# traveller59/second.pytorch

Measured on AMD Instinct MI355X. Metric: frames/sec VoxelNet fwd (car.fhd, ~16k active voxels), higher is better.
Workload: dtype bf16; 1 GPU; car.fhd.config VoxelNet forward (voxelise+VFE+SpMiddleFHD+RPNV2+rotated NMS), inference, batch=8 synthetic KITTI clouds/GPU (17000 pts, 16000 voxels each), random-init weights, inputs resident in HBM; parallelism=frame-dp1, launch_mode=graph, graph_branches=1, steps_in_flight=4, rpn_segments_serialized=True, rulebook_numbering=sorted, points_per_frame=17000

## Files before the change

second.pytorch_amd/csrc/dense.hip:

```cpp
#include "common.hpp"
#include <type_traits>
#include <stdio.h>
#include <stdlib.h>
#include <stdlib.h>

namespace sec {

template <typename T> __device__ __forceinline__ float to_f(T v);
template <> __device__ __forceinline__ float to_f(__hip_bfloat16 v) { return __bfloat162float(v); }
template <> __device__ __forceinline__ float to_f(__half v) { return __half2float(v); }
template <typename T> __device__ __forceinline__ T from_f(float v);
template <> __device__ __forceinline__ __hip_bfloat16 from_f(float v) { return __float2bfloat16(v); }
template <> __device__ __forceinline__ __half from_f(float v) { return __float2half_rn(v); }

template <typename T>
__global__ __launch_bounds__(kBlock) void k_bias_act16(T *__restrict__ x, const float *__restrict__ bias, long long n_vec,
                                                      int c_vec, int relu) {
    for (long long g = (long long)blockIdx.x * kBlock + threadIdx.x; g < n_vec; g += (long long)gridDim.x * kBlock) {
        uint4 v = reinterpret_cast<uint4 *>(x)[g];
        T *e = reinterpret_cast<T *>(&v);
        const float *b = bias + (size_t)(g % c_vec) * 8;
#pragma unroll
        for (int i = 0; i < 8; ++i) {
            float f = to_f<T>(e[i]) + b[i];
// ... 7 lines not shown
__global__ __launch_bounds__(kBlock) void k_bias_act32(float *__restrict__ x, const float *__restrict__ bias, long long n_vec,
                                                      int c_vec, int relu) {
    for (long long g = (long long)blockIdx.x * kBlock + threadIdx.x; g < n_vec; g += (long long)gridDim.x * kBlock) {
        float4 v = reinterpret_cast<float4 *>(x)[g];
        const float *b = bias + (size_t)(g % c_vec) * 4;
        v.x += b[0]; v.y += b[1]; v.z += b[2]; v.w += b[3];
        if (relu) { v.x = fmaxf(v.x, 0.f); v.y = fmaxf(v.y, 0.f); v.z = fmaxf(v.z, 0.f); v.w = fmaxf(v.w, 0.f); }
        reinterpret_cast<float4 *>(x)[g] = v;
    }
}

typedef float f32x16d __attribute__((ext_vector_type(16)));
typedef __bf16 bf16x8d __attribute__((ext_vector_type(8)));
typedef _Float16 f16x8d __attribute__((ext_vector_type(8)));
template <typename T> struct MfmaD;
template <> struct MfmaD<__hip_bfloat16> {
    static __device__ __forceinline__ f32x16d run(uint4 a, uint4 b, f32x16d c) {
        return __builtin_amdgcn_mfma_f32_32x32x16_bf16(__builtin_bit_cast(bf16x8d, a), __builtin_bit_cast(bf16x8d, b), c, 0, 0, 0);
    }
};
template <> struct MfmaD<__half> {
    static __device__ __forceinline__ f32x16d run(uint4 a, uint4 b, f32x16d c) {
        return __builtin_amdgcn_mfma_f32_32x32x16_f16(__builtin_bit_cast(f16x8d, a), __builtin_bit_cast(f16x8d, b), c, 0, 0, 0);
    }
};


typedef float f32x2d __attribute__((ext_vector_type(2)));
template <typename T> __device__ __forceinline__ unsigned pack2(float a, float b);
template <> __device__ __forceinline__ unsigned pack2<__hip_bfloat16>(float a, float b) {
    typedef __bf16 bf16x2d __attribute__((ext_vector_type(2)));
    const f32x2d v = {a, b};
    return __builtin_bit_cast(unsigned, __builtin_convertvector(v, bf16x2d));
}
template <> __device__ __forceinline__ unsigned pack2<__half>(float a, float b) {
    typedef _Float16 f16x2d __attribute__((ext_vector_type(2)));
    const f32x2d v = {a, b};
    return __builtin_bit_cast(unsigned, __builtin_convertvector(v, f16x2d));
}

template <typename T> __device__ __forceinline__ uint2 pack4(float a, float b, float c, float d) {
    T t[4] = {from_f<T>(a), from_f<T>(b), from_f<T>(c), from_f<T>(d)};
    uint2 u;
    __builtin_memcpy(&u, t, 8);
    return u;
}
// ... 184 lines not shown
#pragma unroll
        for (int mt = 0; mt < 2; ++mt) {
            const long long pix0 = m0 + wm * 64 + mt * 32 + 4 * hh;
            T *yp = y + (size_t)pix0 * ldc + co;
#pragma unroll
            for (int i = 0; i < 16; ++i) {
                const int ro = (i & 3) + 8 * (i >> 2);
                if (pix0 + ro < p.m) {
                    float v = acc[mt][nt][i] + bv;
                    if (p.relu) v = v > 0.0f ? v : 0.0f;
                    yp[(size_t)ro * ldc] = from_f<T>(v);
                }
            }
        }
    }
}

template <int N> __device__ __forceinline__ void wait_vmcnt() { asm volatile("s_waitcnt vmcnt(%0)" ::"n"(N) : "memory"); }
__device__ __forceinline__ void lds_barrier() { asm volatile("s_waitcnt lgkmcnt(0)\n\ts_barrier" ::: "memory"); }

template <int CH, int HW_, bool COLKEY> __device__ __forceinline__ int halo_key(int hp) {
    return (COLKEY && CH == 16) ? ((hp % HW_) & 15) : (hp & (CH - 1));
}

#ifdef SEC_CONV2D_EXPERIMENTS
#include "../../tools/kernel_experiments/dense_conv2d_ab.inc"
#endif

template <typename T, int CIN, int TH, int ROLL = 0, bool GATHER = false, int NSPLIT = 1, bool X3 = false, bool TAIL = false>
__global__ __launch_bounds__(256, CIN == 128 ? 3 : 2) void k_conv2d_halo_reg(const T *__restrict__ x, const T *__restrict__ wpk,
                                                            const float *__restrict__ bias, T *__restrict__ y,
                                                            Conv2dParams p, int tiles_y, int tiles_x, int per_xcd,
                                                            const int *__restrict__ site_map, unsigned feat_bytes,
                                                            const unsigned short *__restrict__ tile_order = nullptr,
                                                            const int *__restrict__ live_counts = nullptr,
                                                            const T *__restrict__ background = nullptr,
                                                            const unsigned short *__restrict__ nbr_masks = nullptr,
                                                            const T *__restrict__ bg_in = nullptr,
                                                            const T *__restrict__ x_lo = nullptr, T *__restrict__ y_lo = nullptr,
                                                            const T *__restrict__ background_lo = nullptr,
                                                            const T *__restrict__ bg_in_lo = nullptr, ConvTailArgs tail = ConvTailArgs{}) {
    static_assert(!GATHER || (ROLL == 2 && CIN == 128), "gather prologue: the shared-row loop on two 64-channel planes");
    static_assert(!TAIL || (ROLL == 2 && CIN == 128 && TH == 8 && !GATHER && NSPLIT == 1 && !X3), "fused 1x1 tail: the lazy list form of the 128-channel conv");
    static_assert(!X3 || (ROLL == 2 && CIN == 128 && TH == 8 && !GATHER && NSPLIT == 1 && std::is_same<T, __hip_bfloat16>::value),
                  "three-pass split-fp32 form: the shared-row bf16 loop");
    constexpr int TW = 16, HW_ = TW + 2, HPIX = (TH + 2) * (TW + 2);
    static_assert(NSPLIT == 1 || (NSPLIT == 2 && ROLL == 0 && !GATHER), "pixel split: the two-stage loop only");
    constexpr int MT = TH * TW / 32 / NSPLIT;
    constexpr int CH = CIN / 8, HENT = HPIX * CH;
    constexpr int KC = CIN / 64, NIT = 9 * KC;
    extern __shared__ __attribute__((aligned(16))) uint4 halo_smem[];
    uint4 *hal = halo_smem;
    const int tid = threadIdx.x, lane = tid & 63, wv = tid >> 6;
    const int r = lane & 31, hh = lane >> 5;
    const int ntile = p.batch * tiles_y * tiles_x;
    const int xcd = blockIdx.x % 8, local = blockIdx.x / 8;
    const int n0 = blockIdx.y * (128 / NSPLIT) + (wv % (4 / NSPLIT)) * 32;
    const int mtb = (wv / (4 / NSPLIT)) * MT;
    constexpr int cin8 = CIN / 8;
    const uint4 *x4 = reinterpret_cast<const uint4 *>(x);
    const uint4 *w4 = reinterpret_cast<const uint4 *>(wpk);
    const uint4 *zero16 = w4 + (size_t)9 * cin8 * p.cout;
    auto issue_halo = [&](int tile) {
        const int b = tile / (tiles_y * tiles_x);
        const int trem = tile - b * tiles_y * tiles_x;
        const int y0 = (trem / tiles_x) * TH, x0 = (trem % tiles_x) * TW;
        for (int i = wv; i < (HENT + 63) / 64; i += 4) {
// ... 2 lines not shown
            const int hp = e / CH, slot = e - hp * CH;
            const int hy = hp / HW_, hx = hp - hy * HW_;
            const int iy = y0 - 1 + hy, ix = x0 - 1 + hx;
            const bool ok = iy >= 0 && iy < p.h && ix >= 0 && ix < p.w;
            const uint4 *src = ok ? x4 + (((long long)b * p.h + iy) * p.w + ix) * cin8 + (slot ^ halo_key<CH, HW_, true>(hp)) : zero16;
            __builtin_amdgcn_global_load_lds((glb_ptr_t)src, (lds_ptr_t)&hal[i * 64], 16, 0, 0);
        }
    };
    auto issue_halo2 = [&](int tile, const T *xsrc) {
        const int b = tile / (tiles_y * tiles_x);
        const int trem = tile - b * tiles_y * tiles_x;
        const int y0 = (trem / tiles_x) * TH, x0 = (trem % tiles_x) * TW;
        const unsigned img_bytes = (unsigned)p.h * (unsigned)p.w * (CIN * 2u);
        const __amdgpu_buffer_rsrc_t xrs = __builtin_amdgcn_make_buffer_rsrc(const_cast<T *>(xsrc) + (size_t)b * p.h * p.w * CIN, 0, (int)img_bytes, 0x00020000);
        const int wvs = __builtin_amdgcn_readfirstlane(wv);
        const unsigned slot = lane & 15;
        const unsigned row_pitch = (unsigned)p.w * (CIN * 2u);
        int hx = wvs * 4 + (lane >> 4);
        unsigned rowoff = (unsigned)((y0 - 1) * p.w + (x0 - 1)) * (CIN * 2u);
#pragma unroll
        for (int t = 0; t < (HENT / 64 + 3) / 4; ++t) {
            const int i = wvs + 4 * t;
            if (i < HENT / 64) {
                const unsigned key = (slot ^ ((unsigned)hx & 15u)) << 4;
                unsigned off = rowoff + ((unsigned)hx << 8) + key;
                const unsigned ix = (unsigned)(x0 - 1 + hx);
                off = ix < (unsigned)p.w ? off : 0xfffffff0u;
                __builtin_amdgcn_raw_ptr_buffer_load_lds(xrs, (lds_ptr_t)&hal[i * 64], 16, off, 0, 0, 0);
            }
            hx += 16;
            const bool wrap = hx >= HW_;
            hx = wrap ? hx - HW_ : hx;
            rowoff = wrap ? rowoff + row_pitch : rowoff;
        }
    };
    auto issue_halo2_lazy = [&](int tile, unsigned nmask, const T *xsrc, const T *bgsrc) {
        const int b = tile / (tiles_y * tiles_x);
        const int trem = tile - b * tiles_y * tiles_x;
        const int y0 = (trem / tiles_x) * TH, x0 = (trem % tiles_x) * TW;
        const unsigned img_bytes = (unsigned)p.h * (unsigned)p.w * (CIN * 2u);
        const __amdgpu_buffer_rsrc_t xrs = __builtin_amdgcn_make_buffer_rsrc(const_cast<T *>(xsrc) + (size_t)b * p.h * p.w * CIN, 0, (int)img_bytes, 0x00020000);
        const __amdgpu_buffer_rsrc_t ers = __builtin_amdgcn_make_buffer_rsrc(const_cast<T *>(bgsrc), 0, (int)img_bytes, 0x00020000);
        const int wvs = __builtin_amdgcn_readfirstlane(wv);
        const unsigned slot = lane & 15;
        const unsigned row_pitch = (unsigned)p.w * (CIN * 2u);
        int hx = wvs * 4 + (lane >> 4), hy = 0;
        unsigned rowoff = (unsigned)((y0 - 1) * p.w + (x0 - 1)) * (CIN * 2u);
#pragma unroll
        for (int t = 0; t < (HENT / 64 + 3) / 4; ++t) {
            const int i = wvs + 4 * t;
            if (i < HENT / 64) {
                const unsigned key = (slot ^ ((unsigned)hx & 15u)) << 4;
                unsigned off = rowoff + ((unsigned)hx << 8) + key;
                const unsigned ix = (unsigned)(x0 - 1 + hx);
                off = ix < (unsigned)p.w ? off : 0xfffffff0u;
                const int ry = hy == 0 ? 0 : (hy == TH + 1 ? 2 : 1), rx = hx == 0 ? 0 : (hx == HW_ - 1 ? 2 : 1);
                if ((nmask >> (ry * 3 + rx)) & 1u) __builtin_amdgcn_raw_ptr_buffer_load_lds(xrs, (lds_ptr_t)&hal[i * 64], 16, off, 0, 0, 0);
                else __builtin_amdgcn_raw_ptr_buffer_load_lds(ers, (lds_ptr_t)&hal[i * 64], 16, off, 0, 0, 0);
            }
            hx += 16;
            const bool wrap = hx >= HW_;
            hx = wrap ? hx - HW_ : hx;
            hy = wrap ? hy + 1 : hy;
            rowoff = wrap ? rowoff + row_pitch : rowoff;
        }
    };
    auto issue_halo_gather = [&](int tile) -> unsigned {
        constexpr int NP = (HENT / 64 + 3) / 4;
        const int b = tile / (tiles_y * tiles_x);
        const int trem = tile - b * tiles_y * tiles_x;
        const int y0 = (trem / tiles_x) * TH, x0 = (trem % tiles_x) * TW;
        const unsigned plane = (unsigned)p.h * (unsigned)p.w;
        const __amdgpu_buffer_rsrc_t mrs = __builtin_amdgcn_make_buffer_rsrc(const_cast<int *>(site_map) + (size_t)b * 2 * plane, 0, (int)(plane * 8u), 0x00020000);
        const __amdgpu_buffer_rsrc_t frs = __builtin_amdgcn_make_buffer_rsrc(const_cast<T *>(x), 0, (int)feat_bytes, 0x00020000);
        const int wvs = __builtin_amdgcn_readfirstlane(wv);
        const unsigned slot = lane & 15;
        int hx = wvs * 4 + (lane >> 4), iy = y0 - 1;
        unsigned rowp1[NP], coff[NP], any = 0;
#pragma unroll
        for (int t = 0; t < NP; ++t) {
            const int i = wvs + 4 * t;
            rowp1[t] = 0;
            coff[t] = 0;
            if (i < HENT / 64) {
                const unsigned c = slot ^ ((unsigned)hx & 15u);
                const int ix = x0 - 1 + hx;
                const bool ok = (unsigned)ix < (unsigned)p.w && (unsigned)iy < (unsigned)p.h;
                const unsigned moff = ((c >> 3 ? plane : 0u) + (unsigned)(iy * p.w + ix)) * 4u;
                rowp1[t] = __builtin_amdgcn_raw_buffer_load_b32(mrs, ok ? moff : 0xfffffffcu, 0, 0);
                coff[t] = (c & 7u) << 4;
            }
            hx += 16;
            const bool wrap = hx >= HW_;
            hx = wrap ? hx - HW_ : hx;
            iy = wrap ? iy + 1 : iy;
        }
#pragma unroll
        for (int t = 0; t < NP; ++t) any |= rowp1[t];
        __shared__ unsigned wave_any[4];
        const unsigned long long bal = __ballot(any != 0);
        if (lane == 0) wave_any[wv] = bal != 0ull;
        __syncthreads();
        if ((wave_any[0] | wave_any[1] | wave_any[2] | wave_any[3]) == 0u) return 0u;
#pragma unroll
        for (int t = 0; t < NP; ++t) {
            const int i = wvs + 4 * t;
            if (i < HENT / 64) {
                const unsigned off = rowp1[t] ? (rowp1[t] - 1u) * (CIN * 1u) + coff[t] : 0xfffffff0u;
// ... 141 lines not shown
            for (int ty_ = 0; ty_ < TH; ++ty_) {
                const int oy = y0 + ty_;
                if (oy < p.h && ox < p.w) y4[(((size_t)b * p.h + oy) * p.w + ox) * (p.cout / 8) + blockIdx.y * 16 + ch] = v;
            }
            return;
        }
    } else if constexpr (ROLL >= 2) {
        if (nbr_masks) issue_halo2_lazy(tile, nmask, x, bg_in);
        else issue_halo2(tile, x);
    } else issue_halo(tile);
#ifdef SEC_CONV_TIMELINE
    long long tl_issue = 0, tl_eb1 = 0, tl_eb2 = 0;
    if (tl) tl_issue = clock64();
#endif
    {
        const int b = tile / (tiles_y * tiles_x);
        const int trem = tile - b * tiles_y * tiles_x;
        const int y0 = (trem / tiles_x) * TH, x0 = (trem % tiles_x) * TW;
        uint4 bq[2][4];
        constexpr int RD = 8;
        uint4 br[RD];
        typedef unsigned int u32x4b __attribute__((ext_vector_type(4)));
        const __amdgpu_buffer_rsrc_t wrs = __builtin_amdgcn_make_buffer_rsrc(const_cast<T *>(wpk), 0, (int)(((X3 ? 18 : 9) * cin8 + 1) * p.cout * 16), 0x00020000);
        const unsigned wvoff = (unsigned)(hh * p.cout + n0 + r) * 16u;
        const unsigned wstep = (unsigned)p.cout * 16u;
        auto ld_b = [&](unsigned chunk) {
            return __builtin_bit_cast(uint4, (u32x4b)__builtin_amdgcn_raw_buffer_load_b128(wrs, wvoff, chunk * wstep, 0));
        };
        if constexpr (ROLL >= 2) {
#pragma unroll
            for (int f = 0; f < RD - 1; ++f) br[f] = ld_b((f % 3) * 48 + (f / 3) * 2);
        } else if constexpr (ROLL) {
#pragma unroll
            for (int f = 0; f < RD - 1; ++f) br[f] = wlane[(size_t)f * 2 * p.cout];
        } else {
            load_b(0, bq[0]);
        }
        f32x16d acc[MT];
#pragma unroll
        for (int a = 0; a < MT; ++a)
#pragma unroll
            for (int i = 0; i < 16; ++i) acc[a][i] = 0.0f;
        __syncthreads();
#ifdef SEC_CONV_TIMELINE
        if (tl) tl1 = clock64();
#endif
        bool live = true;
        if constexpr (GATHER) live = gather_live != 0;
        else if (p.zskip) {
            unsigned nz = 0;
            for (int e = tid; e < HENT; e += 256) {
                const uint4 v = hal[e];
                nz |= v.x | v.y | v.z | v.w;
            }
            live = __syncthreads_or((int)(nz != 0)) != 0;
        }
        uint4 af[2][MT];
        int tap = 0, kc = 0;
        if (live && !ROLL) load_a(0, 0, 0, af[0]);
        if constexpr (ROLL >= 2) {
            static_assert(ROLL < 2 || (KC == 2 && CH == 16 && TH == 8), "8 k-steps per tap, rows (mt, mt + 4)");
            const char *halb = reinterpret_cast<const char *>(hal);
            const int colr = r & 15;
            const unsigned base0 = (unsigned)((r >> 4) * 4 * HW_ + colr) * (CH * 16);
            uint4 fr[2][6];
            auto load_f2 = [&](unsigned bdx, unsigned key, int cidx, int j0, uint4 (&dst)[6]) {
                const unsigned a = bdx + (((unsigned)cidx << 4) ^ key);
#pragma unroll
                for (int j = j0; j < j0 + 2; ++j) dst[j] = *reinterpret_cast<const uint4 *>(halb + a + j * HW_ * (CH * 16));
            };
            auto frag_off = [](int j) { return (j % 3) * 48 + (j / 3) * 2; };
            if (live) {
                constexpr int NPASS = X3 ? 3 : 1;
#pragma unroll 1
                for (int pass = 0; pass < NPASS; ++pass) {
                    const unsigned wp = (X3 && pass == 1) ? 9u * cin8 : 0u;
                    if (X3 && pass > 0) {
                        if (pass == 2) {
                            __syncthreads();
                            if (nbr_masks) issue_halo2_lazy(tile, nmask, x_lo, bg_in_lo);
                            else issue_halo2(tile, x_lo);
                        }
#pragma unroll
// ... 73 lines not shown
            if (nkc == KC) { nkc = 0; ++ntap; }
#pragma unroll
            for (int s = 0; s < 4; ++s) {
                if (s < 3) load_a(tap, kc, s + 1, af[(s + 1) & 1]);
                else if (it + 1 < NIT) load_a(ntap, nkc, 0, af[0]);
#pragma unroll
                for (int mt = 0; mt < MT; ++mt) acc[mt] = MfmaD<T>::run(bq[cur][s], af[s & 1][mt], acc[mt]);
            }
            tap = ntap;
            kc = nkc;
        }
#ifdef SEC_CONV_TIMELINE
        if (tl) tl2 = clock64();
#endif
        if constexpr (CIN == 128 && TH == 8) {
            constexpr int PITCH = 17;
            __syncthreads();
#ifdef SEC_CONV_TIMELINE
            if (tl) tl_eb1 = clock64();
#endif
            uint4 *ot = halo_smem;
            float4 bv[4];
#pragma unroll
            for (int g = 0; g < 4; ++g) bv[g] = bias ? *reinterpret_cast<const float4 *>(bias + n0 + 8 * g + 4 * hh) : make_float4(0.0f, 0.0f, 0.0f, 0.0f);
            auto put_tile = [&](auto relu_tag, auto lo_tag) {
                constexpr bool RELU = decltype(relu_tag)::value;
                constexpr bool LOW = decltype(lo_tag)::value;
#pragma unroll
                for (int mt = 0; mt < MT; ++mt) {
                    unsigned lo[4], hi[4];
#pragma unroll
                    for (int g = 0; g < 4; ++g) {
                        float v[4] = {acc[mt][4 * g] + bv[g].x, acc[mt][4 * g + 1] + bv[g].y, acc[mt][4 * g + 2] + bv[g].z, acc[mt][4 * g + 3] + bv[g].w};
                        if (RELU) {
#pragma unroll
                            for (int j = 0; j < 4; ++j) v[j] = __builtin_fmaxf(v[j], 0.0f);
                        }
                        lo[g] = pack2<T>(v[0], v[1]);
                        hi[g] = pack2<T>(v[2], v[3]);
                        if constexpr (LOW) {
                            lo[g] = pack2<T>(v[0] - __uint_as_float(lo[g] << 16), v[1] - __uint_as_float(lo[g] & 0xffff0000u));
                            hi[g] = pack2<T>(v[2] - __uint_as_float(hi[g] << 16), v[3] - __uint_as_float(hi[g] & 0xffff0000u));
                        }
                    }
                    const int q = ROLL >= 2 ? (mt + 4 * (r >> 4)) * 16 + (r & 15) : mt * 32 + r;
#pragma unroll
                    for (int pr = 0; pr < 2; ++pr) {
                        const auto sx = __builtin_amdgcn_permlane32_swap(lo[2 * pr], lo[2 * pr + 1], false, false);
                        const auto sy = __builtin_amdgcn_permlane32_swap(hi[2 * pr], hi[2 * pr + 1], false, false);
                        ot[q * PITCH + wv * 4 + 2 * pr + hh] = make_uint4(sx[0], sy[0], sx[1], sy[1]);
// ... 150 lines not shown
                                  const unsigned short *nbr_masks = nullptr, const void *bg_in = nullptr,
                                  const void *x_lo = nullptr, void *y_lo = nullptr, const void *background_lo = nullptr,
                                  const void *bg_in_lo = nullptr, const ConvTailArgs &tail = ConvTailArgs{}) {
    constexpr size_t lds_tile = (size_t)(TH + 2) * 18 * (CIN / 8) * 16;
    const long lds_pad = 0;
    const size_t lds = lds_tile + (size_t)lds_pad;
    static bool configured = false;
    auto fn = k_conv2d_halo_reg<T, CIN, TH, ROLL, GATHER, NSPLIT, X3, TAIL>;
    if (!configured) {
        (void)hipFuncSetAttribute(reinterpret_cast<const void *>(fn), hipFuncAttributeMaxDynamicSharedMemorySize, (int)lds);
        configured = true;
    }
    const int ty = div_up(p.h, TH), tx = div_up(p.w, 16);
    const int per_xcd = div_up(p.batch * ty * tx, 8);
    const int gx = per_xcd * 8;
    if (TAIL) set_last_kernel("k_conv2d_halo_reg<%s, %d, %d, %d, false, 1, false, true>", dtype_name<T>(), CIN, TH, ROLL);
    else if (X3) set_last_kernel("k_conv2d_halo_reg<%s, %d, %d, %d, false, 1, true>", dtype_name<T>(), CIN, TH, ROLL);
    else if (NSPLIT == 1) set_last_kernel("k_conv2d_halo_reg<%s, %d, %d, %d, %s>", dtype_name<T>(), CIN, TH, ROLL, GATHER ? "true" : "false");
    else set_last_kernel("k_conv2d_halo_reg<%s, %d, %d, %d, %s, %d>", dtype_name<T>(), CIN, TH, ROLL, GATHER ? "true" : "false", NSPLIT);
    hipLaunchKernelGGL(fn, dim3(gx, p.cout / (128 / NSPLIT)), dim3(256), lds, st, (const T *)x, (const T *)wpk, bias, (T *)y, p, ty, tx, per_xcd,
                       site_map, feat_bytes, tile_order, live_counts, (const T *)background, nbr_masks, (const T *)bg_in, (const T *)x_lo, (T *)y_lo,
                       (const T *)background_lo, (const T *)bg_in_lo, tail);
    return check_launch();
}

template <typename T, int BN, int TPW>
__global__ __launch_bounds__(kBlock) void k_conv1x1_nhwc(const T *__restrict__ x, const T *__restrict__ wpk,
                                                        const float *__restrict__ bias, T *__restrict__ y, Conv2dParams p) {
    constexpr int BM = 128, NTW = BN / 64, CC = 2;
    constexpr int PERB = BN * 8 / kBlock;
    __shared__ uint4 sA[2][BM * 8];
    __shared__ uint4 sB[CC][8 * BN];
    const int tid = threadIdx.x, lane = tid & 63, wv = tid >> 6;
    const int r = lane & 31, hh = lane >> 5;
    const int wm = wv & 1, wn = wv >> 1;
    const int n0 = blockIdx.y * BN;
    const int cin8 = p.cin / 8;
    const uint4 *x4 = reinterpret_cast<const uint4 *>(x);
    const uint4 *w4 = reinterpret_cast<const uint4 *>(wpk);
    const uint4 *zero16 = w4 + (size_t)cin8 * p.cout;
    const long long tile0 = (long long)blockIdx.x * TPW;
    const long long ntiles = (p.m + BM - 1) / BM;
    if (tile0 >= ntiles) return;
    const int nt_local = (int)((ntiles - tile0 < TPW) ? ntiles - tile0 : TPW);
    const int slot = lane & 7;
    auto issue_a = [&](int it, int buf) {
// ... 390 lines not shown
}

#include "dense_patch.hpp"

static bool conv2d_patch_enabled() {
    static int v = -1;
    if (v < 0) {
        const char *e = getenv("SEC_CONV2D_PATCH");
        v = (e && *e == '0') ? 0 : 1;
    }
    return v != 0;
}

template <typename T>
static int launch_conv2d(const void *x, const void *wpk, const float *bias, void *y, const Conv2dParams &p, hipStream_t st) {
    dim3 block(kBlock);
    if (conv2d_variant() == 13 && conv2d_patch_enabled()) {
        const int rc = patch::dispatch<T>(x, wpk, bias, y, p, p.cout, st);
        if (rc != patch::kNotTaken) return rc;
    }
    if (conv2d_variant() == 14 && p.ksize == 3 && p.stride == 1 && p.pad == 1 && p.cout % 128 == 0 && p.cin == 128)
        return launch_conv2d_halo_reg<T, 128, 8>(x, wpk, bias, y, p, st);
    if (conv2d_variant() == 13 && p.ksize == 3 && p.stride == 1 && p.pad == 1 && p.cout % 128 == 0 && (p.cin == 128 || p.cin == 64))
        return p.cin == 128 ? launch_conv2d_halo_reg<T, 128, 8, 2>(x, wpk, bias, y, p, st) : launch_conv2d_halo_reg<T, 64, 8>(x, wpk, bias, y, p, st);
    if (conv2d_variant() == 13 && p.ksize == 3 && p.stride == 1 && p.pad == 1 && p.cout % 128 == 0 && p.cin == 256)
        return launch_conv2d_halo_reg<T, 256, 4>(x, wpk, bias, y, p, st);
    if (conv2d_variant() == 13 && p.ksize == 3 && p.stride == 1 && p.pad == 1 && p.cout == 64 && p.cin == 64)
        return launch_conv2d_halo_reg<T, 64, 8, 0, false, 2>(x, wpk, bias, y, p, st);
    if (conv2d_variant() == 15 && p.ksize == 3 && p.stride == 1 && p.pad == 1 && p.cout % 128 == 0 && p.cin == 128)
        return launch_conv2d_halo_reg<T, 128, 8, 1>(x, wpk, bias, y, p, st);
#ifdef SEC_CONV2D_EXPERIMENTS
    if (conv2d_variant() >= 5 && conv2d_variant() <= 12 && p.ksize == 3 && p.stride == 1 && p.pad == 1 && p.cout % 128 == 0 &&
        (p.cin == 128 || p.cin == 64)) {
#define SEC_HALO_PIPE(NQ_, KS_, NB_, CK_, FP_)                                                                  \
    return p.cin == 128 ? launch_conv2d_halo_pipe<T, 128, 8, NQ_, KS_, NB_, CK_, FP_>(x, wpk, bias, y, p, st)   \
                        : launch_conv2d_halo_pipe<T, 64, 8, NQ_, KS_, NB_, CK_, FP_>(x, wpk, bias, y, p, st)
        switch (conv2d_variant()) {
        case 5: SEC_HALO_PIPE(4, 64, 2, false, false);
        case 8: SEC_HALO_PIPE(2, 64, 2, true, false);
        case 10: SEC_HALO_PIPE(4, 64, 2, true, false);
        case 11: SEC_HALO_PIPE(4, 64, 2, false, true);
        default: SEC_HALO_PIPE(4, 64, 2, true, true);
        }
#undef SEC_HALO_PIPE
    }
    if (conv2d_variant() >= 2 && conv2d_variant() <= 4 && p.ksize == 3 && p.stride == 1 && p.pad == 1 &&
        p.cout % 128 == 0 && (p.cin == 128 || p.cin == 64)) {
// ... 200 lines not shown
                              void *workspace, size_t workspace_bytes, void *stream) {
    return rpn_tile_live_impl(site_map, batch, h, w, layers, tile_order, live_counts, nullptr, workspace, workspace_bytes, stream);
}

SEC_API int sec_rpn_tile_live_masks(const int *site_map, int batch, int h, int w, int layers, unsigned short *tile_order, int *live_counts,
                                    unsigned short *nbr_masks, void *workspace, size_t workspace_bytes, void *stream) {
    if (!nbr_masks) return SEC_E_INVALID;
    return rpn_tile_live_impl(site_map, batch, h, w, layers, tile_order, live_counts, nbr_masks, workspace, workspace_bytes, stream);
}

static int conv2d_tiles_impl(const void *x, int batch, int h, int w, const void *packed_weight, const float *bias, int cout, int relu,
                             const unsigned short *tile_order, const int *live_counts, const void *background,
                             const unsigned short *nbr_masks, const void *background_in, void *y, int dtype, void *stream) {
    if (!x || !packed_weight || !y || batch <= 0 || h <= 0 || w <= 0 || (tile_order && !live_counts)) return SEC_E_INVALID;
    if (cout % 128 || (dtype != SEC_BF16 && dtype != SEC_F16)) return SEC_E_UNSUPPORTED;
    apply_list_threshold_env();
    Conv2dParams p;
    p.batch = batch; p.h = h; p.w = w; p.cin = 128; p.cout = cout; p.ksize = 3; p.stride = 1; p.pad = 1;
    p.relu = relu & 1; p.zskip = 0; p.stagger = 0;
    p.ho = h; p.wo = w;
    p.m = (long long)batch * h * w;
    hipStream_t st = (hipStream_t)stream;
    if (dtype == SEC_BF16)
        return launch_conv2d_halo_reg<__hip_bfloat16, 128, 8, 2>(x, packed_weight, bias, y, p, st, nullptr, 0, tile_order, live_counts, background,
                                                                 nbr_masks, background_in);
    return launch_conv2d_halo_reg<__half, 128, 8, 2>(x, packed_weight, bias, y, p, st, nullptr, 0, tile_order, live_counts, background, nbr_masks,
                                                     background_in);
}

SEC_API int sec_conv2d_nhwc_tiles(const void *x, int batch, int h, int w, const void *packed_weight, const float *bias, int cout,
                                  int relu, const unsigned short *tile_order, const int *live_counts, const void *background,
                                  void *y, int dtype, void *stream) {
    if (tile_order && !background) return SEC_E_INVALID;
    return conv2d_tiles_impl(x, batch, h, w, packed_weight, bias, cout, relu, tile_order, live_counts, background, nullptr, nullptr, y, dtype,
                             stream);
}

SEC_API int sec_conv2d_nhwc_tiles_lazy(const void *x, int batch, int h, int w, const void *packed_weight, const float *bias, int cout,
                                       int relu, const unsigned short *tile_order, const int *live_counts, const void *background,
                                       const unsigned short *nbr_masks, const void *background_in, void *y, int dtype, void *stream) {
    if (!tile_order || !nbr_masks || !background_in) return SEC_E_INVALID;
    return conv2d_tiles_impl(x, batch, h, w, packed_weight, bias, cout, relu, tile_order, live_counts, background, nbr_masks, background_in, y,
                             dtype, stream);
}

SEC_API int sec_conv2d_nhwc_tiles_tail(const void *x, int batch, int h, int w, const void *packed_weight, const float *bias, int relu,
                                       const unsigned short *tile_order, const int *live_counts, const unsigned short *nbr_masks,
                                       const void *background_in, const void *packed_w1, const float *bias1, int relu1, const void *packed_w2,
                                       const float *bias2, int cout2, void *y_heads, int dtype, void *stream) {
    if (!x || !packed_weight || !tile_order || !live_counts || !nbr_masks || !background_in || !packed_w1 || !bias1 || !packed_w2 || !y_heads ||
        batch <= 0 || h <= 0 || w <= 0)
        return SEC_E_INVALID;
    if (cout2 != 64 || (dtype != SEC_BF16 && dtype != SEC_F16)) return SEC_E_UNSUPPORTED;
    apply_list_threshold_env();
    Conv2dParams p;
    p.batch = batch; p.h = h; p.w = w; p.cin = 128; p.cout = 128; p.ksize = 3; p.stride = 1; p.pad = 1;
    p.relu = relu & 1; p.zskip = 0; p.stagger = 0;
    p.ho = h; p.wo = w;
    p.m = (long long)batch * h * w;
    const ConvTailArgs tail{packed_w1, packed_w2, bias1, bias2, y_heads, relu1 & 1};
    hipStream_t st = (hipStream_t)stream;
    if (dtype == SEC_BF16)
        return launch_conv2d_halo_reg<__hip_bfloat16, 128, 8, 2, false, 1, false, true>(x, packed_weight, bias, nullptr, p, st, nullptr, 0, tile_order, live_counts,
                                                                                       nullptr, nbr_masks, background_in, nullptr, nullptr, nullptr, nullptr, tail);
    return launch_conv2d_halo_reg<__half, 128, 8, 2, false, 1, false, true>(x, packed_weight, bias, nullptr, p, st, nullptr, 0, tile_order, live_counts, nullptr,
                                                                           nbr_masks, background_in, nullptr, nullptr, nullptr, nullptr, tail);
}

SEC_API size_t sec_conv2d_packed_weight_bytes(int cout, int cin, int ksize, int dtype) {
    if (dtype == SEC_F32 || cout <= 0 || cin <= 0 || cin % 64 || cout % 64 || ksize <= 0) return 0;
    return (size_t)ksize * ksize * cin * cout * 2 + 16;
}

SEC_API int sec_conv2d_pack_weight(const void *weight, int cout, int cin, int ksize, int dtype, void *packed, void *stream) {
    if (!weight || !packed || sec_conv2d_packed_weight_bytes(cout, cin, ksize, dtype) == 0) return SEC_E_INVALID;
    long long total = (long long)ksize * ksize * cin * cout;
    hipStream_t st = (hipStream_t)stream;
    if (hipMemsetAsync((char *)packed + total * 2, 0, 16, st) != hipSuccess) return SEC_E_LAUNCH;
    if (dtype == SEC_BF16)
        hipLaunchKernelGGL(k_conv2d_pack<__hip_bfloat16>, dim3(div_up(total, kBlock)), dim3(kBlock), 0, st,
                           (const __hip_bfloat16 *)weight, cout, cin, ksize, (__hip_bfloat16 *)packed);
    else
        hipLaunchKernelGGL(k_conv2d_pack<__half>, dim3(div_up(total, kBlock)), dim3(kBlock), 0, st, (const __half *)weight,
                           cout, cin, ksize, (__half *)packed);
    return check_launch();
}

SEC_API int sec_conv2d_nhwc(const void *x, int batch, int h, int w, int cin, const void *packed_weight, const float *bias,
// ... 84 lines not shown
    if (blocks > 256 * 32) blocks = 256 * 32;
    hipLaunchKernelGGL(k_split_bf16x2, dim3((unsigned)blocks), dim3(kBlock), 0, (hipStream_t)stream, (const float4 *)x, n / 4, (uint2 *)hi, (uint2 *)lo);
    return check_launch();
}

SEC_API int sec_merge_bf16x2_f32(const void *hi, const void *lo, long long n, float *y, void *stream) {
    if (n < 0 || n % 4 || (n > 0 && (!y || !hi || !lo))) return SEC_E_INVALID;
    if (n == 0) return SEC_OK;
    long long blocks = div_up(n / 4, kBlock);
    if (blocks > 256 * 32) blocks = 256 * 32;
    hipLaunchKernelGGL(k_merge_bf16x2, dim3((unsigned)blocks), dim3(kBlock), 0, (hipStream_t)stream, (const uint2 *)hi, (const uint2 *)lo, n / 4, (float4 *)y);
    return check_launch();
}

SEC_API int sec_conv2d_nhwc_x3(const void *x_hi, const void *x_lo, int batch, int h, int w, const void *packed_weight_hi_lo, const float *bias,
                               int cout, int relu, void *y_hi, void *y_lo, void *stream) {
    if (!x_hi || !x_lo || !packed_weight_hi_lo || !y_hi || !y_lo || batch <= 0 || h <= 0 || w <= 0) return SEC_E_INVALID;
    if (cout % 128 || (long long)h * w * 256 >= (1ll << 31)) return SEC_E_UNSUPPORTED;
    Conv2dParams p;
    p.batch = batch; p.h = h; p.w = w; p.cin = 128; p.cout = cout; p.ksize = 3; p.stride = 1; p.pad = 1;
    p.relu = relu & 1; p.zskip = (relu >> 1) & 1; p.stagger = 0;
    p.ho = h; p.wo = w;
    p.m = (long long)batch * h * w;
    return launch_conv2d_halo_reg<__hip_bfloat16, 128, 8, 2, false, 1, true>(x_hi, packed_weight_hi_lo, bias, y_hi, p, (hipStream_t)stream, nullptr, 0,
                                                                              nullptr, nullptr, nullptr, nullptr, nullptr, x_lo, y_lo);
}

SEC_API int sec_conv2d_nhwc_x3_tiles(const void *x_hi, const void *x_lo, int batch, int h, int w, const void *packed_weight_hi_lo,
                                     const float *bias, int cout, int relu, const unsigned short *tile_order, const int *live_counts,
                                     const void *background_hi, const void *background_lo, const unsigned short *nbr_masks,
                                     const void *background_in_hi, const void *background_in_lo, void *y_hi, void *y_lo, void *stream) {
    if (!x_hi || !x_lo || !packed_weight_hi_lo || !y_hi || !y_lo || !tile_order || !live_counts || batch <= 0 || h <= 0 || w <= 0) return SEC_E_INVALID;
    if ((background_hi == nullptr) != (background_lo == nullptr)) return SEC_E_INVALID;
    if (nbr_masks && (!background_in_hi || !background_in_lo)) return SEC_E_INVALID;
    if (cout % 128 || (long long)h * w * 256 >= (1ll << 31)) return SEC_E_UNSUPPORTED;
    apply_list_threshold_env();
    Conv2dParams p;
    p.batch = batch; p.h = h; p.w = w; p.cin = 128; p.cout = cout; p.ksize = 3; p.stride = 1; p.pad = 1;
    p.relu = relu & 1; p.zskip = 0; p.stagger = 0;
    p.ho = h; p.wo = w;
    p.m = (long long)batch * h * w;
    return launch_conv2d_halo_reg<__hip_bfloat16, 128, 8, 2, false, 1, true>(x_hi, packed_weight_hi_lo, bias, y_hi, p, (hipStream_t)stream, nullptr, 0,
                                                                              tile_order, live_counts, background_hi, nbr_masks, background_in_hi,
                                                                              x_lo, y_lo, background_lo, background_in_lo);
}

SEC_API int sec_conv2d_nhwc_gather(const void *features, long long feature_rows, const int *site_map, int batch, int h, int w,
                                   const void *packed_weight, const float *bias, int cout, int relu, const unsigned short *tile_order,
                                   const int *live_counts, const void *background, void *y, int dtype, void *stream) {
    if (!site_map || !packed_weight || !y || batch <= 0 || h <= 0 || w <= 0 || feature_rows < 0 || (!features && feature_rows > 0)) return SEC_E_INVALID;
    if (tile_order && !live_counts) return SEC_E_INVALID;
    if (cout % 128 || (dtype != SEC_BF16 && dtype != SEC_F16) || feature_rows * 128 >= (1ll << 31) ||
        (long long)h * w * 8 >= (1ll << 31)) return SEC_E_UNSUPPORTED;
    apply_list_threshold_env();
    Conv2dParams p;
    p.batch = batch; p.h = h; p.w = w; p.cin = 128; p.cout = cout; p.ksize = 3; p.stride = 1; p.pad = 1;
    p.relu = relu & 1; p.zskip = 0; p.stagger = 0;
    p.ho = h; p.wo = w;
    p.m = (long long)batch * h * w;
    hipStream_t st = (hipStream_t)stream;
    const unsigned fb = (unsigned)(feature_rows * 128);
    if (dtype == SEC_BF16)
        return launch_conv2d_halo_reg<__hip_bfloat16, 128, 8, 2, true>(features, packed_weight, bias, y, p, st, site_map, fb, tile_order, live_counts, background);
    return launch_conv2d_halo_reg<__half, 128, 8, 2, true>(features, packed_weight, bias, y, p, st, site_map, fb, tile_order, live_counts, background);
}

SEC_API int sec_conv1x1_chain_nhwc(const void *x, long long pixels, const void *packed_w1, const float *bias1, int relu1,
                                   const void *packed_w2, const float *bias2, int cout2, void *y, int dtype, void *stream) {
    if (!x || !packed_w1 || !packed_w2 || !bias1 || !y || pixels < 0) return SEC_E_INVALID;
    if ((cout2 != 64 && cout2 != 128) || (dtype != SEC_BF16 && dtype != SEC_F16)) return SEC_E_UNSUPPORTED;
    if (pixels == 0) return SEC_OK;
    hipStream_t st = (hipStream_t)stream;
    if (dtype == SEC_BF16)
        return launch_conv1x1_chain<__hip_bfloat16>(x, pixels, packed_w1, bias1, packed_w2, bias2, cout2, relu1, y, st);
    return launch_conv1x1_chain<__half>(x, pixels, packed_w1, bias1, packed_w2, bias2, cout2, relu1, y, st);
}

SEC_API int sec_conv1x1_chain_x3(const void *x_hi, const void *x_lo, long long pixels, const void *packed_w1_hi_lo, const float *bias1, int relu1,
                                 const void *packed_w2_hi_lo, const float *bias2, int cout2, float *y, void *stream) {
    if (!x_hi || !x_lo || !packed_w1_hi_lo || !packed_w2_hi_lo || !bias1 || !y || pixels < 0) return SEC_E_INVALID;
    if (cout2 != 64 && cout2 != 128) return SEC_E_UNSUPPORTED;
    if (pixels == 0) return SEC_OK;
    hipStream_t st = (hipStream_t)stream;
    const int blocks = (int)div_up(pixels, 128);
    if (cout2 == 64)
        hipLaunchKernelGGL((k_conv1x1_chain_x3<1>), dim3(blocks), dim3(256), 0, st, (const __hip_bfloat16 *)x_hi, (const __hip_bfloat16 *)x_lo,
                           (const __hip_bfloat16 *)packed_w1_hi_lo, bias1, (const __hip_bfloat16 *)packed_w2_hi_lo, bias2, y, pixels, relu1);
// ... 41 lines not shown
```

Baseline: 21660 frames/s.

## Add 16x16x32 MFMA path for 128-channel halo conv and make it default

```diff
diff --git a/second.pytorch_amd/csrc/dense.hip b/second.pytorch_amd/csrc/dense.hip
--- a/second.pytorch_amd/csrc/dense.hip
+++ b/second.pytorch_amd/csrc/dense.hip
@@ -53,6 +53,18 @@
 template <> struct MfmaD<__half> {
     static __device__ __forceinline__ f32x16d run(uint4 a, uint4 b, f32x16d c) {
         return __builtin_amdgcn_mfma_f32_32x32x16_f16(__builtin_bit_cast(f16x8d, a), __builtin_bit_cast(f16x8d, b), c, 0, 0, 0);
+    }
+};
+typedef float f32x4d __attribute__((ext_vector_type(4)));
+template <typename T> struct MfmaK32;
+template <> struct MfmaK32<__hip_bfloat16> {
+    static __device__ __forceinline__ f32x4d run(uint4 a, uint4 b, f32x4d c) {
+        return __builtin_amdgcn_mfma_f32_16x16x32_bf16(__builtin_bit_cast(bf16x8d, a), __builtin_bit_cast(bf16x8d, b), c, 0, 0, 0);
+    }
+};
+template <> struct MfmaK32<__half> {
+    static __device__ __forceinline__ f32x4d run(uint4 a, uint4 b, f32x4d c) {
+        return __builtin_amdgcn_mfma_f32_16x16x32_f16(__builtin_bit_cast(f16x8d, a), __builtin_bit_cast(f16x8d, b), c, 0, 0, 0);
     }
 };
 
@@ -283,6 +295,7 @@
 template <int CH, int HW_, bool COLKEY> __device__ __forceinline__ int halo_key(int hp) {
     return (COLKEY && CH == 16) ? ((hp % HW_) & 15) : (hp & (CH - 1));
 }
+template <int ROLL> __device__ __forceinline__ unsigned halo_colkey(unsigned hx) { return ROLL == 3 ? (2u * hx) & 15u : hx & 15u; }
 
 #ifdef SEC_CONV2D_EXPERIMENTS
 #include "../../tools/kernel_experiments/dense_conv2d_ab.inc"
@@ -301,9 +314,9 @@
                                                             const T *__restrict__ x_lo = nullptr, T *__restrict__ y_lo = nullptr,
                                                             const T *__restrict__ background_lo = nullptr,
                                                             const T *__restrict__ bg_in_lo = nullptr, ConvTailArgs tail = ConvTailArgs{}) {
-    static_assert(!GATHER || (ROLL == 2 && CIN == 128), "gather prologue: the shared-row loop on two 64-channel planes");
-    static_assert(!TAIL || (ROLL == 2 && CIN == 128 && TH == 8 && !GATHER && NSPLIT == 1 && !X3), "fused 1x1 tail: the lazy list form of the 128-channel conv");
-    static_assert(!X3 || (ROLL == 2 && CIN == 128 && TH == 8 && !GATHER && NSPLIT == 1 && std::is_same<T, __hip_bfloat16>::value),
+    static_assert(!GATHER || (ROLL >= 2 && CIN == 128), "gather prologue: the shared-row loop on two 64-channel planes");
+    static_assert(!TAIL || (ROLL >= 2 && CIN == 128 && TH == 8 && !GATHER && NSPLIT == 1 && !X3), "fused 1x1 tail: the lazy list form of the 128-channel conv");
+    static_assert(!X3 || (ROLL >= 2 && CIN == 128 && TH == 8 && !GATHER && NSPLIT == 1 && std::is_same<T, __hip_bfloat16>::value),
                   "three-pass split-fp32 form: the shared-row bf16 loop");
     constexpr int TW = 16, HW_ = TW + 2, HPIX = (TH + 2) * (TW + 2);
     static_assert(NSPLIT == 1 || (NSPLIT == 2 && ROLL == 0 && !GATHER), "pixel split: the two-stage loop only");
@@ -352,7 +365,7 @@
         for (int t = 0; t < (HENT / 64 + 3) / 4; ++t) {
             const int i = wvs + 4 * t;
             if (i < HENT / 64) {
-                const unsigned key = (slot ^ ((unsigned)hx & 15u)) << 4;
+                const unsigned key = (slot ^ halo_colkey<ROLL>((unsigned)hx)) << 4;
                 unsigned off = rowoff + ((unsigned)hx << 8) + key;
                 const unsigned ix = (unsigned)(x0 - 1 + hx);
                 off = ix < (unsigned)p.w ? off : 0xfffffff0u;
@@ -380,7 +393,7 @@
         for (int t = 0; t < (HENT / 64 + 3) / 4; ++t) {
             const int i = wvs + 4 * t;
             if (i < HENT / 64) {
-                const unsigned key = (slot ^ ((unsigned)hx & 15u)) << 4;
+                const unsigned key = (slot ^ halo_colkey<ROLL>((unsigned)hx)) << 4;
                 unsigned off = rowoff + ((unsigned)hx << 8) + key;
                 const unsigned ix = (unsigned)(x0 - 1 + hx);
                 off = ix < (unsigned)p.w ? off : 0xfffffff0u;
@@ -413,7 +426,7 @@
             rowp1[t] = 0;
             coff[t] = 0;
             if (i < HENT / 64) {
-                const unsigned c = slot ^ ((unsigned)hx & 15u);
+                const unsigned c = slot ^ halo_colkey<ROLL>((unsigned)hx);
                 const int ix = x0 - 1 + hx;
                 const bool ok = (unsigned)ix < (unsigned)p.w && (unsigned)iy < (unsigned)p.h;
                 const unsigned moff = ((c >> 3 ? plane : 0u) + (unsigned)(iy * p.w + ix)) * 4u;
@@ -601,12 +614,32 @@
         uint4 br[RD];
         typedef unsigned int u32x4b __attribute__((ext_vector_type(4)));
         const __amdgpu_buffer_rsrc_t wrs = __builtin_amdgcn_make_buffer_rsrc(const_cast<T *>(wpk), 0, (int)(((X3 ? 18 : 9) * cin8 + 1) * p.cout * 16), 0x00020000);
-        const unsigned wvoff = (unsigned)(hh * p.cout + n0 + r) * 16u;
+        const unsigned wvoff = ROLL == 3 ? (unsigned)((lane >> 4) * p.cout + n0 + (lane & 15)) * 16u : (unsigned)(hh * p.cout + n0 + r) * 16u;
         const unsigned wstep = (unsigned)p.cout * 16u;
         auto ld_b = [&](unsigned chunk) {
             return __builtin_bit_cast(uint4, (u32x4b)__builtin_amdgcn_raw_buffer_load_b128(wrs, wvoff, chunk * wstep, 0));
         };
-        if constexpr (ROLL >= 2) {
+        auto ld_w = [&](unsigned chunk, int g) {
+            return __builtin_bit_cast(uint4, (u32x4b)__builtin_amdgcn_raw_buffer_load_b128(wrs, wvoff + (unsigned)g * 256u, chunk * wstep, 0));
+        };
+        uint4 wb[ROLL == 3 ? 2 : 1][3][2];
+        f32x4d acc3[ROLL == 3 ? TH : 1][2];
+        auto prime_w = [&](unsigned wp) {
+#pragma unroll
+            for (int g = 0; g < 2; ++g) {
+#pragma unroll
+                for (int dy = 0; dy < 3; ++dy) wb[0][dy][g] = ld_w(wp + dy * 48, g);
+#pragma unroll
+                for (int dy = 0; dy < 2; ++dy) wb[ROLL == 3][dy][g] = ld_w(wp + dy * 48 + 4, g);
+            }
+        };
+        if constexpr (ROLL == 3) {
+#pragma unroll
+            for (int y = 0; y < TH; ++y)
+#pragma unroll
+                for (int g = 0; g < 2; ++g) acc3[y][g] = f32x4d{0.0f, 0.0f, 0.0f, 0.0f};
+            prime_w(0u);
+        } else if constexpr (ROLL >= 2) {
 #pragma unroll
             for (int f = 0; f < RD - 1; ++f) br[f] = ld_b((f % 3) * 48 + (f / 3) * 2);
         } else if constexpr (ROLL) {
@@ -637,7 +670,72 @@
         uint4 af[2][MT];
         int tap = 0, kc = 0;
         if (live && !ROLL) load_a(0, 0, 0, af[0]);
-        if constexpr (ROLL >= 2) {
+        if constexpr (ROLL == 3) {
+            static_assert(KC == 2 && CH == 16 && TH == 8, "4 k32 steps per tap, ten halo rows");
+            const char *halb = reinterpret_cast<const char *>(hal);
+            const unsigned pxl = lane & 15, kq = lane >> 4;
+            constexpr unsigned ROWB = HW_ * CH * 16;
+            auto f_addr = [&](int dx, int k32) {
+                return (pxl + (unsigned)dx) * (CH * 16) + (((unsigned)k32 << 6) ^ ((kq ^ halo_colkey<3>(pxl + (unsigned)dx)) << 4));
+            };
+            uint4 fr[4];
+            if (live) {
+                constexpr int NPASS = X3 ? 3 : 1;
+#pragma unroll 1
+                for (int pass = 0; pass < NPASS; ++pass) {
+                    const unsigned wp = (X3 && pass == 1) ? 9u * cin8 : 0u;
+                    if (X3 && pass > 0) {
+                        if (pass == 2) {
+                            __syncthreads();
+                            if (nbr_masks) issue_halo2_lazy(tile, nmask, x_lo, bg_in_lo);
+                            else issue_halo2(tile, x_lo);
+                        }
+                        prime_w(wp);
+                        if (pass == 2) __syncthreads();
+                    }
+                    {
+                        const unsigned a0 = f_addr(0, 0);
+#pragma unroll
+                        for (int h = 0; h < 3; ++h) fr[h] = *reinterpret_cast<const uint4 *>(halb + a0 + h * ROWB);
+                    }
+#pragma unroll 1
+                    for (int dx = 0; dx < 3; ++dx) {
+                        const int dxn = dx < 2 ? dx + 1 : 2;
+                        const unsigned fb[2] = {(pxl + (unsigned)dx) * (CH * 16), (pxl + (unsigned)dxn) * (CH * 16)};
+                        const unsigned fk[2] = {(kq ^ halo_colkey<3>(pxl + (unsigned)dx)) << 4, (kq ^ halo_colkey<3>(pxl + (unsigned)dxn)) << 4};
+                        auto fa = [&](int k) { return fb[k >> 2] + (((unsigned)(k & 3) << 6) ^ fk[k >> 2]); };
+                        const unsigned ct = wp + dx * 16, cn = wp + dxn * 16;
+#pragma unroll
+                        for (int k32 = 0; k32 < 4; ++k32) {
+#pragma unroll
+                            for (int hy = 0; hy < TH + 2; ++hy) {
+                                const int t = k32 * (TH + 2) + hy, cur = k32 & 1;
+                                const unsigned c1 = k32 < 3 ? ct + 4 * (k32 + 1) : cn;
+                                const unsigned c2 = k32 < 2 ? ct + 4 * (k32 + 2) : cn + 4 * (k32 - 2);
+                                if (hy == 0 || hy >= TH) {
+                                    const int dyl = hy == 0 ? 2 : hy - TH;
+#pragma unroll
+                                    for (int g = 0; g < 2; ++g) wb[hy == 0 ? cur ^ 1 : cur][dyl][g] = ld_w((hy == 0 ? c1 : c2) + dyl * 48, g);
+                                }
+                                {
+                                    const int tn = t + 3;
+                                    fr[tn & 3] = *reinterpret_cast<const uint4 *>(halb + fa(tn / (TH + 2)) + (tn % (TH + 2)) * ROWB);
+                                }
+#pragma unroll
+                                for (int dy = 0; dy < 3; ++dy) {
+                                    const int y = hy - dy;
+                                    if (y < 0 || y >= TH) continue;
+#pragma unroll
+                                    for (int g = 0; g < 2; ++g) acc3[y][g] = MfmaK32<T>::run(wb[cur][dy][g], fr[t & 3], acc3[y][g]);
+                                }
+                                __builtin_amdgcn_sched_barrier(0);
+                            }
+                        }
+                    }
+                }
+            }
+            live = false;
+        } else if constexpr (ROLL >= 2) {
             static_assert(ROLL < 2 || (KC == 2 && CH == 16 && TH == 8), "8 k-steps per tap, rows (mt, mt + 4)");
             const char *halb = reinterpret_cast<const char *>(hal);
             const int colr = r & 15;
@@ -757,10 +855,38 @@
             uint4 *ot = halo_smem;
             float4 bv[4];
 #pragma unroll
-            for (int g = 0; g < 4; ++g) bv[g] = bias ? *reinterpret_cast<const float4 *>(bias + n0 + 8 * g + 4 * hh) : make_float4(0.0f, 0.0f, 0.0f, 0.0f);
+            for (int g = 0; g < 4; ++g)
+                bv[g] = bias ? *reinterpret_cast<const float4 *>(bias + n0 + (ROLL == 3 ? 16 * (g & 1) + 4 * (lane >> 4) : 8 * g + 4 * hh)) : make_float4(0.0f, 0.0f, 0.0f, 0.0f);
             auto put_tile = [&](auto relu_tag, auto lo_tag) {
                 constexpr bool RELU = decltype(relu_tag)::value;
                 constexpr bool LOW = decltype(lo_tag)::value;
+                if constexpr (ROLL == 3) {
+                    const int kq = lane >> 4;
+#pragma unroll
+                    for (int y = 0; y < TH; ++y) {
+                        unsigned lo[2], hi[2];
+#pragma unroll
+                        for (int g = 0; g < 2; ++g) {
+                            const float4 b4 = bv[g];
+                            float v[4] = {acc3[y][g][0] + b4.x, acc3[y][g][1] + b4.y, acc3[y][g][2] + b4.z, acc3[y][g][3] + b4.w};
+                            if (RELU) {
+#pragma unroll
+                                for (int j = 0; j < 4; ++j) v[j] = __builtin_fmaxf(v[j], 0.0f);
+                            }
+                            lo[g] = pack2<T>(v[0], v[1]);
+                            hi[g] = pack2<T>(v[2], v[3]);
+                            if constexpr (LOW) {
+                                lo[g] = pack2<T>(v[0] - __uint_as_float(lo[g] << 16), v[1] - __uint_as_float(lo[g] & 0xffff0000u));
+                                hi[g] = pack2<T>(v[2] - __uint_as_float(hi[g] << 16), v[3] - __uint_as_float(hi[g] & 0xffff0000u));
+                            }
+                        }
+                        const auto sx = __builtin_amdgcn_permlane16_swap(lo[0], lo[1], false, false);
+                        const auto sy = __builtin_amdgcn_permlane16_swap(hi[0], hi[1], false, false);
+                        ot[(y * 16 + (lane & 15)) * PITCH + wv * 4 + 2 * (kq & 1) + (kq >> 1)] = make_uint4(sx[0], sy[0], sx[1], sy[1]);
+                        __builtin_amdgcn_sched_barrier(0);
+                    }
+                    return;
+                }
 #pragma unroll
                 for (int mt = 0; mt < MT; ++mt) {
                     unsigned lo[4], hi[4];
@@ -957,6 +1083,20 @@
                        site_map, feat_bytes, tile_order, live_counts, (const T *)background, nbr_masks, (const T *)bg_in, (const T *)x_lo, (T *)y_lo,
                        (const T *)background_lo, (const T *)bg_in_lo, tail);
     return check_launch();
+}
+
+static int conv2d_c128_roll() {
+    static int v = -1;
+    if (v < 0) {
+        const char *e = getenv("SEC_CONV2D_MFMA");
+        v = (e && atoi(e) == 32) ? 2 : 3;
+    }
+    return v;
+}
+template <typename T, bool GATHER = false, bool X3 = false, bool TAIL = false, typename... A>
+static int launch_conv2d_c128(A... a) {
+    return conv2d_c128_roll() == 3 ? launch_conv2d_halo_reg<T, 128, 8, 3, GATHER, 1, X3, TAIL>(a...)
+                                   : launch_conv2d_halo_reg<T, 128, 8, 2, GATHER, 1, X3, TAIL>(a...);
 }
 
 template <typename T, int BN, int TPW>
@@ -1393,7 +1533,7 @@
     if (conv2d_variant() == 14 && p.ksize == 3 && p.stride == 1 && p.pad == 1 && p.cout % 128 == 0 && p.cin == 128)
         return launch_conv2d_halo_reg<T, 128, 8>(x, wpk, bias, y, p, st);
     if (conv2d_variant() == 13 && p.ksize == 3 && p.stride == 1 && p.pad == 1 && p.cout % 128 == 0 && (p.cin == 128 || p.cin == 64))
-        return p.cin == 128 ? launch_conv2d_halo_reg<T, 128, 8, 2>(x, wpk, bias, y, p, st) : launch_conv2d_halo_reg<T, 64, 8>(x, wpk, bias, y, p, st);
+        return p.cin == 128 ? launch_conv2d_c128<T>(x, wpk, bias, y, p, st) : launch_conv2d_halo_reg<T, 64, 8>(x, wpk, bias, y, p, st);
     if (conv2d_variant() == 13 && p.ksize == 3 && p.stride == 1 && p.pad == 1 && p.cout % 128 == 0 && p.cin == 256)
         return launch_conv2d_halo_reg<T, 256, 4>(x, wpk, bias, y, p, st);
     if (conv2d_variant() == 13 && p.ksize == 3 && p.stride == 1 && p.pad == 1 && p.cout == 64 && p.cin == 64)
@@ -1640,9 +1780,9 @@
     p.m = (long long)batch * h * w;
     hipStream_t st = (hipStream_t)stream;
     if (dtype == SEC_BF16)
-        return launch_conv2d_halo_reg<__hip_bfloat16, 128, 8, 2>(x, packed_weight, bias, y, p, st, nullptr, 0, tile_order, live_counts, background,
+        return launch_conv2d_c128<__hip_bfloat16>(x, packed_weight, bias, y, p, st, nullptr, 0, tile_order, live_counts, background,
                                                                  nbr_masks, background_in);
-    return launch_conv2d_halo_reg<__half, 128, 8, 2>(x, packed_weight, bias, y, p, st, nullptr, 0, tile_order, live_counts, background, nbr_masks,
+    return launch_conv2d_c128<__half>(x, packed_weight, bias, y, p, st, nullptr, 0, tile_order, live_counts, background, nbr_masks,
                                                      background_in);
 }
 
@@ -1679,9 +1819,9 @@
     const ConvTailArgs tail{packed_w1, packed_w2, bias1, bias2, y_heads, relu1 & 1};
     hipStream_t st = (hipStream_t)stream;
     if (dtype == SEC_BF16)
-        return launch_conv2d_halo_reg<__hip_bfloat16, 128, 8, 2, false, 1, false, true>(x, packed_weight, bias, nullptr, p, st, nullptr, 0, tile_order, live_counts,
+        return launch_conv2d_c128<__hip_bfloat16, false, false, true>(x, packed_weight, bias, nullptr, p, st, nullptr, 0, tile_order, live_counts,
                                                                                        nullptr, nbr_masks, background_in, nullptr, nullptr, nullptr, nullptr, tail);
-    return launch_conv2d_halo_reg<__half, 128, 8, 2, false, 1, false, true>(x, packed_weight, bias, nullptr, p, st, nullptr, 0, tile_order, live_counts, nullptr,
+    return launch_conv2d_c128<__half, false, false, true>(x, packed_weight, bias, nullptr, p, st, nullptr, 0, tile_order, live_counts, nullptr,
                                                                            nbr_masks, background_in, nullptr, nullptr, nullptr, nullptr, tail);
 }
 
@@ -1812,7 +1952,7 @@
     p.relu = relu & 1; p.zskip = (relu >> 1) & 1; p.stagger = 0;
     p.ho = h; p.wo = w;
     p.m = (long long)batch * h * w;
-    return launch_conv2d_halo_reg<__hip_bfloat16, 128, 8, 2, false, 1, true>(x_hi, packed_weight_hi_lo, bias, y_hi, p, (hipStream_t)stream, nullptr, 0,
+    return launch_conv2d_c128<__hip_bfloat16, false, true>(x_hi, packed_weight_hi_lo, bias, y_hi, p, (hipStream_t)stream, nullptr, 0,
                                                                               nullptr, nullptr, nullptr, nullptr, nullptr, x_lo, y_lo);
 }
 
@@ -1830,7 +1970,7 @@
     p.relu = relu & 1; p.zskip = 0; p.stagger = 0;
     p.ho = h; p.wo = w;
     p.m = (long long)batch * h * w;
-    return launch_conv2d_halo_reg<__hip_bfloat16, 128, 8, 2, false, 1, true>(x_hi, packed_weight_hi_lo, bias, y_hi, p, (hipStream_t)stream, nullptr, 0,
+    return launch_conv2d_c128<__hip_bfloat16, false, true>(x_hi, packed_weight_hi_lo, bias, y_hi, p, (hipStream_t)stream, nullptr, 0,
                                                                               tile_order, live_counts, background_hi, nbr_masks, background_in_hi,
                                                                               x_lo, y_lo, background_lo, background_in_lo);
 }
@@ -1851,8 +1991,8 @@
     hipStream_t st = (hipStream_t)stream;
     const unsigned fb = (unsigned)(feature_rows * 128);
     if (dtype == SEC_BF16)
-        return launch_conv2d_halo_reg<__hip_bfloat16, 128, 8, 2, true>(features, packed_weight, bias, y, p, st, site_map, fb, tile_order, live_counts, background);
-    return launch_conv2d_halo_reg<__half, 128, 8, 2, true>(features, packed_weight, bias, y, p, st, site_map, fb, tile_order, live_counts, background);
+        return launch_conv2d_c128<__hip_bfloat16, true>(features, packed_weight, bias, y, p, st, site_map, fb, tile_order, live_counts, background);
+    return launch_conv2d_c128<__half, true>(features, packed_weight, bias, y, p, st, site_map, fb, tile_order, live_counts, background);
 }
 
 SEC_API int sec_conv1x1_chain_nhwc(const void *x, long long pixels, const void *packed_w1, const float *bias1, int relu1,
```

Result: faster. 22210 frames/s, median of 6 (+2.6%).
